# manonkok/Rao-Blackwellized-SLAM-smoothing

Hardware: AMD Instinct MI355X
Metric: particle-steps/s (filter) + smoother wall-clock, N=65k T=3k (higher is better)
Workload: dtype f64

## Files before the change

### rao-blackwellized-slam-smoothing_amd/csrc/rbpf_step_sym.hip

```cpp
#include <type_traits>
#include "rbpf_internal.hpp"
#include "rbpf_device.hpp"
#include "rbpf_model_dev.hpp"

#ifdef RBPF_STAMPS
#define RBPF_SYM_KSTAMP(k) if (blockIdx.x == 4000 && threadIdx.x == 0 && a.stamps) a.stamps[k] = __builtin_amdgcn_s_memrealtime()
#else
#define RBPF_SYM_KSTAMP(k)
#endif
#ifndef RBPF_SYM_LIGHT_WGS
#define RBPF_SYM_LIGHT_WGS 2
#endif

namespace rbpf {

typedef double dbl2s __attribute__((ext_vector_type(2)));
typedef float flt2s __attribute__((ext_vector_type(2)));
typedef float flt4s __attribute__((ext_vector_type(4)));
template <typename TS> struct SymTile { static constexpr int cg = 2; };
template <> struct SymTile<float> { static constexpr int cg = 4; };

template <typename TS> __device__ __forceinline__ dbl2s ld_tile(const TS* p);
template <> __device__ __forceinline__ dbl2s ld_tile<double>(const double* p) { return *reinterpret_cast<const dbl2s*>(p); }
template <> __device__ __forceinline__ dbl2s ld_tile<float>(const float* p) {
// ... 214 lines not shown
  constexpr int UP = UP0 * NPH > kSymStage / 2 ? kSymStage / 2 / NPH : UP0;
  constexpr int PB = (WR || UP < 4) ? 2 : 4;
  constexpr bool kCol = !(DIAG && NACT == 1);
  constexpr bool kF4 = std::is_same<TS, float>::value;
  static_assert(!kF4 || (NPH == 1 && UP % 2 == 0 && PB == 2), "fp32 tiles: whole column quads per round");
  for (int p0 = pbeg + cp; p0 < pbeg + kSymStage / 2; p0 += UP * NPH) {
    dbl2s v[UP][NACT];
    if constexpr (kF4) {
      flt4s raw[UP / 2][NACT];
#pragma unroll
      for (int j = 0; j < UP / 2; ++j)
#pragma unroll
        for (int q = 0; q < NACT; ++q) raw[j][q] = *reinterpret_cast<const flt4s*>(src[Q0 + q] + (size_t)((p0 >> 1) + j) * (4 * kSymChunk));
#pragma unroll
      for (int j = 0; j < UP / 2; ++j)
#pragma unroll
        for (int q = 0; q < NACT; ++q) {
          v[2 * j][q].x = (double)raw[j][q].x; v[2 * j][q].y = (double)raw[j][q].y;
          v[2 * j + 1][q].x = (double)raw[j][q].z; v[2 * j + 1][q].y = (double)raw[j][q].w;
        }
    } else {
#pragma unroll
    for (int u = 0; u < UP; ++u)
#pragma unroll
      for (int q = 0; q < NACT; ++q) v[u][q] = ld_tile<TS>(src[Q0 + q] + (size_t)(p0 + u * NPH) * (2 * kSymChunk));
    }
#pragma unroll
    for (int hh = 0; hh < UP / PB; ++hh) {
      double pc[PB][2][DE];
      dbl2s outv[kF4 && WR ? PB : 1][NACT];
#pragma unroll
      for (int uu = 0; uu < PB; ++uu) {
        const int u = hh * PB + uu, p = p0 + u * NPH;
        double h0[DE], h1[DE];
        {
          double hb[2 * DE + 2];
#pragma unroll
          for (int k2 = 0; k2 < (2 * DE + 1) / 2; ++k2) {
            const dbl2s t = *reinterpret_cast<const dbl2s*>(Hc + (size_t)p * 2 * DE + 2 * k2);
            hb[2 * k2] = t.x; hb[2 * k2 + 1] = t.y;
          }
#pragma unroll
          for (int k = 0; k < DE; ++k) { h0[k] = hb[k]; h1[k] = hb[DE + k]; }
        }
#pragma unroll
        for (int e = 0; e < 2; ++e)
#pragma unroll
          for (int k = 0; k < DE; ++k) pc[uu][e][k] = 0.0;
        constexpr int kChunk = 4 * D, NCH = (ND + kChunk - 1) / kChunk;
        double kc0[kChunk], kc1[kChunk];
        double pq0[NACT], pq1[NACT];
#pragma unroll
        for (int q = 0; q < NACT; ++q) { pq0[q] = v[u][q].x; pq1[q] = v[u][q].y; }
        if (WR && NCH == 1 && ND > 0) {
          double ca[D], cb[D], na[D], nb_[D];
#pragma unroll
          for (int k = 0; k < D; ++k) {
            const dbl2s t = *reinterpret_cast<const dbl2s*>(kst + ((size_t)(p % (kSymStage / 2)) * ND + k) * 2);
            ca[k] = t.x; cb[k] = t.y;
          }
#pragma unroll
          for (int s = 0; s < NS; ++s) {
            if (s + 1 < NS) {
#pragma unroll
              for (int k = 0; k < D; ++k) {
                const dbl2s t = *reinterpret_cast<const dbl2s*>(kst + ((size_t)(p % (kSymStage / 2)) * ND + (s + 1) * D + k) * 2);
                na[k] = t.x; nb_[k] = t.y;
              }
            }
#pragma unroll
            for (int q = 0; q < NACT; ++q)
#pragma unroll
              for (int k = 0; k < D; ++k) {
                pq0[q] = fma(-ks[KR == 1 ? 0 : Q0 + q][s * D + k], ca[k], pq0[q]);
                pq1[q] = fma(-ks[KR == 1 ? 0 : Q0 + q][s * D + k], cb[k], pq1[q]);
              }
            if (s + 1 < NS) {
              __builtin_amdgcn_sched_barrier(0);
#pragma unroll
              for (int k = 0; k < D; ++k) { ca[k] = na[k]; cb[k] = nb_[k]; }
            }
          }
        }
#pragma unroll
        for (int q = 0; q < NACT; ++q) {
          double p0v = pq0[q], p1v = pq1[q];
          if (WR) {
            if (NCH == 1) {
            } else {
#pragma unroll
              for (int ch = 0; ch < NCH; ++ch) {
#pragma unroll
                for (int k = 0; k < kChunk; ++k) {
                  if (ch * kChunk + k < ND) {
                    const dbl2s t = *reinterpret_cast<const dbl2s*>(kst + ((size_t)(p % (kSymStage / 2)) * ND + ch * kChunk + k) * 2);
                    kc0[k] = t.x; kc1[k] = t.y;
                  }
                }
#pragma unroll
                for (int k = 0; k < kChunk; ++k)
                  if (ch * kChunk + k < ND) {
                    p0v = fma(-ks[KR == 1 ? 0 : Q0 + q][ch * kChunk + k], kc0[k], p0v); p1v = fma(-ks[KR == 1 ? 0 : Q0 + q][ch * kChunk + k], kc1[k], p1v);
                  }
                if (ch + 1 < NCH) __builtin_amdgcn_sched_barrier(0);
              }
            }
            dbl2s o; o.x = p0v; o.y = p1v;
            if constexpr (kF4) outv[uu][q] = o;
            else st_tile<TS>(dst[Q0 + q] + (size_t)p * (2 * kSymChunk), o);
          }
#pragma unroll
          for (int k = 0; k < DE; ++k) accr[Q0 + q][k] = fma(p1v, h1[k], fma(p0v, h0[k], accr[Q0 + q][k]));
          if (!(DIAG && q == 0)) {
#pragma unroll
            for (int k = 0; k < DE; ++k) { pc[uu][0][k] = fma(p0v, hown[Q0 + q][k], pc[uu][0][k]); pc[uu][1][k] = fma(p1v, hown[Q0 + q][k], pc[uu][1][k]); }
          }
        }
      }
      if constexpr (kF4 && WR) {
#pragma unroll
        for (int q = 0; q < NACT; ++q) {
          flt4s o4; o4.x = (float)outv[0][q].x; o4.y = (float)outv[0][q].y; o4.z = (float)outv[1][q].x; o4.w = (float)outv[1][q].y;
          __builtin_nontemporal_store(o4, reinterpret_cast<flt4s*>(dst[Q0 + q] + (size_t)((p0 + hh * PB) >> 1) * (4 * kSymChunk)));
        }
      }
      if (kCol) {
        const int rho = lane >> 4;
#pragma unroll
        for (int g = 0; g < PB / 2; ++g)
#pragma unroll
          for (int k = 0; k < DE; ++k) {
            const double r = wave_sum4(pc[2 * g][0][k], pc[2 * g][1][k], pc[2 * g + 1][0][k], pc[2 * g + 1][1][k]);
            if ((lane & 15) == 0) {
              double* cq = &colp[(size_t)k * ldc + 2 * (p0 + (hh * PB + 2 * g + (rho & 1)) * NPH) + (rho >> 1)];
              *cq = ADD ? *cq + r : r;
            }
          }
      }
    }
  }
}

#ifndef RBPF_SYM_QUAD
#define RBPF_SYM_QUAD 1
#endif
#ifndef RBPF_SYM_QUAD_EMAX
#define RBPF_SYM_QUAD_EMAX 1
#endif
#ifndef RBPF_SYM_QUAD_LOADS
#define RBPF_SYM_QUAD_LOADS 16
#endif
#ifndef RBPF_SYM_BUTTERFLY
#define RBPF_SYM_BUTTERFLY 1
#endif
template <typename TS, int D, int DE, int NACT, bool DIAG, int Q0, int QL = RBPF_SYM_QUAD_LOADS>
__device__ __forceinline__ void sym_block_quad(const TS* const (&src)[kSymRows], const double* __restrict__ Hc,
                                               const double (&hown)[kSymRows][4][DE], double (&accr)[kSymRows][4][DE],
                                               double* __restrict__ colp, int ldc, int lane) {
  const int r16 = lane & 15, g = lane >> 4;
  constexpr bool kCol = !(DIAG && NACT == 1);
  constexpr int TQ = ((DE > 3 ? 8 : QL) / 4) / NACT;
  auto quad = [&](const dbl2s (&vq)[NACT][4], const int t) {
      double h0[DE], h1[DE];
      {
        double hb[2 * DE + 2];
#pragma unroll
        for (int k2 = 0; k2 < (2 * DE + 1) / 2; ++k2) {
          const dbl2s tt = *reinterpret_cast<const dbl2s*>(Hc + (size_t)(4 * t + g) * 2 * DE + 2 * k2);
          hb[2 * k2] = tt.x; hb[2 * k2 + 1] = tt.y;
        }
#pragma unroll
        for (int k = 0; k < DE; ++k) { h0[k] = hb[k]; h1[k] = hb[DE + k]; }
      }
      double pc[2][DE];
#pragma unroll
      for (int e = 0; e < 2; ++e)
#pragma unroll
        for (int k = 0; k < DE; ++k) pc[e][k] = 0.0;
#pragma unroll
      for (int q = 0; q < NACT; ++q)
#pragma unroll
        for (int rq = 0; rq < 4; ++rq) {
          const double p0v = vq[q][rq].x, p1v = vq[q][rq].y;
#pragma unroll
          for (int k = 0; k < DE; ++k) accr[Q0 + q][rq][k] = fma(p1v, h1[k], fma(p0v, h0[k], accr[Q0 + q][rq][k]));
          if (!(DIAG && q == 0)) {
#pragma unroll
            for (int k = 0; k < DE; ++k) { pc[0][k] = fma(p0v, hown[Q0 + q][rq][k], pc[0][k]); pc[1][k] = fma(p1v, hown[Q0 + q][rq][k], pc[1][k]); }
          }
        }
      if (kCol) {
        if constexpr (DE == 3 && RBPF_SYM_BUTTERFLY) {
          __builtin_amdgcn_sched_barrier(0);
          const unsigned b0 = 0u - (unsigned)(lane & 1), b1 = 0u - (unsigned)((lane >> 1) & 1);
          const double r0 = bfly_pair<0x121>(pc[0][0], pc[0][1], b0), r1 = bfly_pair<0x121>(pc[0][2], pc[1][0], b0);
          double w = bfly_pair<0x121>(pc[1][1], pc[1][2], b0);
          double q = bfly_pair<0x122>(r0, r1, b1);
          w += dpp_mov<0x122>(w);
          q += dpp_mov<0x124>(q); w += dpp_mov<0x124>(w);
          q += dpp_mov<0x128>(q); w += dpp_mov<0x128>(w);
          const int col = 2 * (4 * t + g);
          if (r16 < 4) colp[(size_t)(r16 == 3 ? 0 : r16) * ldc + col + (r16 == 3 ? 1 : 0)] = q;
          if (r16 < 2) colp[(size_t)(1 + r16) * ldc + col + 1] = w;
          __builtin_amdgcn_sched_barrier(0);
        } else {
#pragma unroll
          for (int e = 0; e < 2; ++e)
#pragma unroll
            for (int k = 0; k < DE; ++k) {
              const double r = row16_sum(pc[e][k]);
              if (r16 == 0) colp[(size_t)k * ldc + 2 * (4 * t + g) + e] = r;
            }
        }
      }
  };
#pragma unroll 1
  for (int t0 = 0; t0 < kSymChunk / 8; t0 += TQ) {
    dbl2s v[TQ][NACT][4];
#pragma unroll
    for (int u = 0; u < TQ; ++u)
#pragma unroll
      for (int q = 0; q < NACT; ++q)
#pragma unroll
        for (int rq = 0; rq < 4; ++rq)
          v[u][q][rq] = ld_tile<TS>(src[Q0 + q] + (size_t)(t0 + u) * (8 * kSymChunk) + rq * 32);
#pragma unroll
    for (int u = 0; u < TQ; ++u) quad(v[u], t0 + u);
  }
}

template <int D, int DE, int NACT, bool DIAG, int Q0>
__device__ __forceinline__ void sym_block_quad_f4(const float* const (&src)[kSymRows], const double* __restrict__ Hc,
                                                  const double (&hown)[kSymRows][4][DE], double (&accr)[kSymRows][4][DE],
                                                  double* __restrict__ colp, int ldc, int lane) {
  static_assert(DE == 3 && RBPF_SYM_BUTTERFLY, "fp32 tiles: the filter");
  const int r16 = lane & 15, g = lane >> 4;
  constexpr bool kCol = !(DIAG && NACT == 1);
#ifndef RBPF_SYM_QUAD_LOADS_F4
#define RBPF_SYM_QUAD_LOADS_F4 8
#endif
  constexpr int TQ = (RBPF_SYM_QUAD_LOADS_F4 / 4) / NACT;
#pragma unroll 1
  for (int t0 = 0; t0 < kSymChunk / 16; t0 += TQ) {
    flt4s v[TQ][NACT][4];
#pragma unroll
    for (int u = 0; u < TQ; ++u)
#pragma unroll
      for (int q = 0; q < NACT; ++q)
#pragma unroll
        for (int rq = 0; rq < 4; ++rq)
          v[u][q][rq] = *reinterpret_cast<const flt4s*>(src[Q0 + q] + (size_t)(t0 + u) * (16 * kSymChunk) + rq * 64);
#pragma unroll
    for (int u = 0; u < TQ; ++u)
#pragma unroll
      for (int h = 0; h < 2; ++h) {
        const int pi = 2 * (4 * (t0 + u) + g) + h;
        __builtin_amdgcn_sched_barrier(0);
        double h0[DE], h1[DE];
        {
          double hb[2 * DE + 2];
#pragma unroll
          for (int k2 = 0; k2 < (2 * DE + 1) / 2; ++k2) {
            const dbl2s tt = *reinterpret_cast<const dbl2s*>(Hc + (size_t)pi * 2 * DE + 2 * k2);
            hb[2 * k2] = tt.x; hb[2 * k2 + 1] = tt.y;
          }
#pragma unroll
          for (int k = 0; k < DE; ++k) { h0[k] = hb[k]; h1[k] = hb[DE + k]; }
        }
        double pc[2][DE];
#pragma unroll
        for (int e = 0; e < 2; ++e)
#pragma unroll
          for (int k = 0; k < DE; ++k) pc[e][k] = 0.0;
#pragma unroll
        for (int q = 0; q < NACT; ++q)
#pragma unroll
          for (int rq = 0; rq < 4; ++rq) {
            const double p0v = (double)(h ? v[u][q][rq].z : v[u][q][rq].x), p1v = (double)(h ? v[u][q][rq].w : v[u][q][rq].y);
#pragma unroll
            for (int k = 0; k < DE; ++k) accr[Q0 + q][rq][k] = fma(p1v, h1[k], fma(p0v, h0[k], accr[Q0 + q][rq][k]));
            if (!(DIAG && q == 0)) {
#pragma unroll
              for (int k = 0; k < DE; ++k) { pc[0][k] = fma(p0v, hown[Q0 + q][rq][k], pc[0][k]); pc[1][k] = fma(p1v, hown[Q0 + q][rq][k], pc[1][k]); }
            }
          }
        if (kCol) {
          __builtin_amdgcn_sched_barrier(0);
          const unsigned b0 = 0u - (unsigned)(lane & 1), b1 = 0u - (unsigned)((lane >> 1) & 1);
          const double r0 = bfly_pair<0x121>(pc[0][0], pc[0][1], b0), r1 = bfly_pair<0x121>(pc[0][2], pc[1][0], b0);
          double w = bfly_pair<0x121>(pc[1][1], pc[1][2], b0);
          double q = bfly_pair<0x122>(r0, r1, b1);
          w += dpp_mov<0x122>(w);
          q += dpp_mov<0x124>(q); w += dpp_mov<0x124>(w);
          q += dpp_mov<0x128>(q); w += dpp_mov<0x128>(w);
          const int col = 2 * pi;
          if (r16 < 4) colp[(size_t)(r16 == 3 ? 0 : r16) * ldc + col + (r16 == 3 ? 1 : 0)] = q;
          if (r16 < 2) colp[(size_t)(1 + r16) * ldc + col + 1] = w;
          __builtin_amdgcn_sched_barrier(0);
        }
      }
  }
}

template <typename TS, int D, int NS, bool WR, int E, int CH>
__device__ __forceinline__ void step_sym_body(const StepArgs& a) {
#include "rbpf_step_sym_body.inc"
// ... 156 lines not shown
```

### rao-blackwellized-slam-smoothing_amd/csrc/rbpf_step_sym_body.inc

```
  const int chv = CH ? CH : a.lay.CH64;
  const int NW = sym_waves(chv), NT = 64 * NW;
  constexpr int NPH = sym_phases(CH);
  constexpr bool kGStrip = (CH == 16 || CH == 0);
  extern __shared__ double smem[];
  constexpr int DE = D + E, ND = NS * D, NDA = ND > 0 ? ND : 1, NSA = NS > 0 ? NS : 1;
  constexpr bool kSplit = WR && NS > 4;
  const ModelDev& M = a.mdl;
  const Layout& Ly = a.lay;
  const int n = Ly.n, nb = Ly.nb, mc = Ly.mc, ldx = Ly.ldx, ldb = Ly.ldb;
  const int pos = xcd_position((int)blockIdx.x, (int)gridDim.x);
  const int* pre_i = a.pre_i + (size_t)pos * kPreInts;
  if (a.phase >= 0 && pre_i[5] != a.phase) return;
  const int i = pre_i[0];
  const int dslot = WR ? pre_i[4] : i;
  const int tid = threadIdx.x, lane = tid & 63, wave = tid >> 6;
  const SymPlan lp = sym_plan(n, DE, ldx, M.ktot, WR ? ND : 0, chv, ((RBPF_SYM_LIGHT_WGS > 2 && !WR && E == 0) || kGStrip) ? 0 : 1);
  double* Hs = smem + lp.off_H + ((nb * DE) & 1);
  double* xls = smem + lp.off_xl;
  double* PHt = smem + lp.off_PHt;
  double* tabS = smem + lp.off_tab;
  double* tabC = tabS + (M.ktot > 0 ? M.ktot : 1);
  double* misc = smem + lp.off_misc;
  double* red = smem + lp.off_red;
#ifdef RBPF_SYM_DIAG_SAMEBASE
  const int ancb = pre_i[2], baseb = pre_i[3] & 63;
#else
  const int ancb = pre_i[2], baseb = pre_i[3];
#endif
  const bool remote = a.rec != nullptr && ancb >= a.n_bank_local;
  const double* recp = remote ? a.rec + (size_t)(ancb - a.n_bank_local) * a.rec_stride : nullptr;
  const bool remoteP = a.rec != nullptr && baseb >= a.n_bank_local;
  const double* recP = remoteP ? a.rec + (size_t)(baseb - a.n_bank_local) * a.rec_stride : nullptr;
  const TS* srcT = remoteP ? reinterpret_cast<const TS*>(recP) : reinterpret_cast<const TS*>(a.Pt_old) + (size_t)baseb * a.Pt_old_stride;
  const TS* srcB = remoteP ? reinterpret_cast<const TS*>(recP + a.rec_off_B) : reinterpret_cast<const TS*>(a.Pb_old) + (size_t)baseb * a.Pb_old_stride;
  const double* srcX = remote ? recp + a.rec_off_X : a.xl_old + (size_t)ancb * a.xl_old_stride;
  const double* Fs[NSA];
#pragma unroll
  for (int s = 0; s < NSA; ++s) Fs[s] = nullptr;
#pragma unroll
  for (int s = 0; s < NS; ++s) {
    if (a.fset[s]) Fs[s] = a.fset[s] + (size_t)pre_i[kPreSet0 + s] * 2 * D * ldx;
    else Fs[s] = remote ? recp + a.rec_off_F : a.F_old + (size_t)ancb * 2 * D * ldx;
  }

  RBPF_SYM_KSTAMP(0);
  const double* pre_d = a.pre_d + (size_t)pos * kPreDoubles;
  const double px0 = pre_d[0], px1 = pre_d[1], px2 = pre_d[2];
  constexpr int kNNPre = 2;
  const int crot = (M.kind == 1) ? 3 : 0;
  auto jcol = [&](int ci) { const int c = ci + crot; return c >= n ? c - n : c; };
  int nnp[kNNPre][3] = {};
  if (a.H_ext == nullptr) {
#pragma unroll
    for (int it = 0; it < kNNPre; ++it)
      if (tid + it * NT < n) H_column_indices(M, jcol(tid + it * NT), nnp[it]);
  }
  constexpr bool kCorr = !WR && NS > 0;
  constexpr int kFPre = NS > 6 ? 2 : 3, kSPre = kFPre;
  double kvp[kCorr ? kFPre : 1][NDA], ksp[kCorr ? kSPre : 1][NDA];
  if constexpr (kCorr) {
#pragma unroll
    for (int it = 0; it < kFPre; ++it)
      if (tid + it * NT < n) {
#pragma unroll
        for (int s = 0; s < NS; ++s)
#pragma unroll
          for (int k = 0; k < D; ++k) kvp[it][s * D + k] = Fs[s][(size_t)(D + k) * ldx + tid + it * NT];
      }
  }
  if (tid < kPreDoubles) misc[tid] = pre_d[tid];
  constexpr bool kXlLds = !(RBPF_SYM_LIGHT_WGS > 2 && !WR && E == 0) && !kGStrip;
  if (kXlLds) for (int c = tid; c < n; c += NT) xls[c] = srcX[c];
  double Riy[D];
  if (E > 0) {
    const double* iv = remote ? recp + a.rec_off_I : a.ivec_old + (size_t)ancb * a.ivec_old_stride;
    for (int c = tid; c < n; c += NT) Hs[c * DE + D] = iv[c];
#pragma unroll
    for (int aa = 0; aa < D; ++aa) {
      double sacc = 0.0;
#pragma unroll
      for (int bb = 0; bb < D; ++bb) sacc = fma(M.Rinv[aa + D * bb], a.y[bb], sacc);
      Riy[aa] = sacc;
    }
  }
  RBPF_SYM_KSTAMP(1);
  for (int q = tid; q < M.ktot; q += NT) basis_table_entry(M, q, px0, px1, px2, tabS, tabC);
  __syncthreads();
  RBPF_SYM_KSTAMP(2);
  {
    auto column = [&](int c, const int* nn) {
      double h[D];
      if (a.H_ext != nullptr) {
#pragma unroll
        for (int k = 0; k < D; ++k) h[k] = a.H_ext[((size_t)i * D + k) * ldx + c];
      } else {
        H_column<D>(M, c, nn, tabS, tabC, &misc[8], h);
      }
#pragma unroll
      for (int k = 0; k < D; ++k) Hs[c * DE + k] = h[k];
      if (E > 0) {
        double sp = Hs[c * DE + D];
#pragma unroll
        for (int k = 0; k < D; ++k) sp = fma(h[k], Riy[k], sp);
#pragma unroll
        for (int k = 0; k < D; ++k) a.Hb_new[((size_t)i * D + k) * ldx + c] = h[k];
        a.ivec_new[(size_t)i * ldx + c] = sp;
      }
    };
#pragma unroll
    for (int it = 0; it < kNNPre; ++it)
      if (tid + it * NT < n) column(jcol(tid + it * NT), nnp[it]);
    for (int ci = tid + kNNPre * NT; ci < n; ci += NT) {
      int nn[3] = {0, 0, 0};
      if (a.H_ext == nullptr) H_column_indices(M, jcol(ci), nn);
      column(jcol(ci), nn);
    }
  }
  __syncthreads();
  if constexpr (kCorr) {
    constexpr int NG = NS * D * DE;
    double g[NG];
#pragma unroll
    for (int q = 0; q < NG; ++q) g[q] = 0.0;
    auto gcol = [&](int c, const double* kv) {
      double h[DE];
#pragma unroll
      for (int k = 0; k < DE; ++k) h[k] = Hs[c * DE + k];
#pragma unroll
      for (int s = 0; s < NS; ++s)
#pragma unroll
        for (int k = 0; k < D; ++k)
#pragma unroll
          for (int j = 0; j < DE; ++j) g[(s * D + k) * DE + j] = fma(kv[s * D + k], h[j], g[(s * D + k) * DE + j]);
    };
#pragma unroll
    for (int it = 0; it < kFPre; ++it)
      if (tid + it * NT < n) gcol(tid + it * NT, kvp[it]);
    for (int c = tid + kFPre * NT; c < n; c += NT) {
      double kv[NDA];
#pragma unroll
      for (int s = 0; s < NS; ++s)
#pragma unroll
        for (int k = 0; k < D; ++k) kv[s * D + k] = Fs[s][(size_t)(D + k) * ldx + c];
      gcol(c, kv);
    }
    wave_sums_packed<NG>(g, lane, [&](int q, double s) { red[wave * kSymRed + q] = s; });
  }

  RBPF_SYM_KSTAMP(3);
  {
  const int rp = (NPH == 1) ? wave : (wave % (chv / 2)), cp = (NPH == 1) ? 0 : (wave / (chv / 2));
  const int rows[kSymRows] = {rp, chv - 1 - rp};
  constexpr bool kQuad = RBPF_SYM_QUAD && !WR && NPH == 1 && E <= RBPF_SYM_QUAD_EMAX;
  constexpr int kQL = CH == 0 ? 8 : RBPF_SYM_QUAD_LOADS;
  double accr[kSymRows][DE], hown[kSymRows][DE], ks[kSplit ? 1 : kSymRows][NDA];
  double accq[kQuad ? kSymRows : 1][4][DE], hq[kQuad ? kSymRows : 1][4][DE];
  if constexpr (kQuad) {
#pragma unroll
    for (int q = 0; q < kSymRows; ++q)
#pragma unroll
      for (int rq = 0; rq < 4; ++rq)
#pragma unroll
        for (int k = 0; k < DE; ++k) { accq[q][rq][k] = 0.0; hq[q][rq][k] = Hs[(nb + rows[q] * kSymChunk + 16 * rq + (lane & 15)) * DE + k]; }
  }
#pragma unroll
  for (int q = 0; q < kSymRows; ++q) {
    const int r = nb + rows[q] * kSymChunk + lane;
#pragma unroll
    for (int k = 0; k < DE; ++k) { accr[q][k] = 0.0; hown[q][k] = Hs[r * DE + k]; }
#pragma unroll
    for (int s = 0; s < NS; ++s)
#pragma unroll
      for (int k = 0; k < D; ++k) ks[kSplit ? 0 : q][s * D + k] = (WR && !kSplit) ? Fs[s][(size_t)k * ldx + r] : 0.0;
    for (int b = 0; b < nb && cp == 0 && !kQuad; ++b) {
      double pv = (double)srcB[(size_t)b * ldb + r];
      if (WR) {
#pragma unroll
        for (int sset = 0; sset < NS; ++sset)
#pragma unroll
          for (int k = 0; k < D; ++k) pv = fma(-Fs[sset][(size_t)k * ldx + b], Fs[sset][(size_t)(D + k) * ldx + r], pv);
      }
#pragma unroll
      for (int k = 0; k < DE; ++k) accr[q][k] = fma(pv, Hs[b * DE + k], accr[q][k]);
    }
  }
  if (WR) __syncthreads();
  {
    TS* dT = reinterpret_cast<TS*>(a.Pt_new) + (size_t)dslot * Ly.szT;
    double* kst = smem + lp.off_kst + (size_t)wave * kSymStage * ND;
    double* colw = (rp == 0) ? PHt + nb : (kGStrip ? smem + lp.off_col1 + (size_t)wave * DE * kSymChunk : smem + sym_off_col(lp.off_col1, DE, chv, rp));
    const int ldc = (rp == 0) ? ldx : (kGStrip ? kSymChunk : sym_ld_col(chv, rp));
    double* gstrip = kGStrip ? a.strip_ws + (size_t)blockIdx.x * a.strip_ws_stride + sym_off_col(0, DE, chv, rp) : nullptr;
    const double* Hcore = Hs + (size_t)nb * DE;
    double kpre[NDA];
    auto fetch = [&](int col0) {
#pragma unroll
      for (int s = 0; s < NS; ++s)
#pragma unroll
        for (int k = 0; k < D; ++k) kpre[s * D + k] = Fs[s][(size_t)(D + k) * ldx + col0 + (lane & (kSymStage - 1))];
    };
    auto park = [&]() {
      asm volatile("" ::: "memory");
      if (lane < kSymStage) {
#pragma unroll
        for (int k = 0; k < ND; ++k) kst[((size_t)(lane >> 1) * ND + k) * 2 + (lane & 1)] = kpre[k];
      }
      asm volatile("" ::: "memory");
    };
    const int last = rows[kSymRows - 1];
    for (int J = 0; J <= last; ++J) {
      const TS* src[kSymRows]; TS* dst[kSymRows];
#pragma unroll
      for (int q = 0; q < kSymRows; ++q) {
        const size_t off = ((size_t)rows[q] * (rows[q] + 1) / 2 + J) * kSymTile + SymTile<TS>::cg * lane;
        src[q] = srcT + off; dst[q] = dT + off;
      }
      const double* Hc = Hcore + (size_t)J * kSymChunk * DE;
      double* colp = (kGStrip && rp > 0) ? colw : colw + (size_t)J * kSymChunk;
      if constexpr (kQuad) {
        const TS* srq[kSymRows];
#pragma unroll
        for (int q = 0; q < kSymRows; ++q)
          srq[q] = srcT + ((size_t)rows[q] * (rows[q] + 1) / 2 + J) * kSymTile + SymTile<TS>::cg * (kSymChunk * (lane >> 4) + (lane & 15));
        if constexpr (std::is_same<TS, float>::value) {
          if (J < rows[0]) sym_block_quad_f4<D, DE, 2, false, 0>(srq, Hc, hq, accq, colp, ldc, lane);
          else if (J == rows[0]) sym_block_quad_f4<D, DE, 2, true, 0>(srq, Hc, hq, accq, colp, ldc, lane);
          else if (J < last) sym_block_quad_f4<D, DE, 1, false, 1>(srq, Hc, hq, accq, colp, ldc, lane);
          else sym_block_quad_f4<D, DE, 1, true, 1>(srq, Hc, hq, accq, colp, ldc, lane);
        } else {
        if (J < rows[0]) sym_block_quad<TS, D, DE, 2, false, 0, kQL>(srq, Hc, hq, accq, colp, ldc, lane);
        else if (J == rows[0]) sym_block_quad<TS, D, DE, 2, true, 0, kQL>(srq, Hc, hq, accq, colp, ldc, lane);
        else if (J < last) sym_block_quad<TS, D, DE, 1, false, 1, kQL>(srq, Hc, hq, accq, colp, ldc, lane);
        else sym_block_quad<TS, D, DE, 1, true, 1, kQL>(srq, Hc, hq, accq, colp, ldc, lane);
        }
      } else if constexpr (!kSplit) {
        for (int pbeg = 0; pbeg < kSymChunk / 2; pbeg += kSymStage / 2) {
          if (WR && ND > 0) { fetch(nb + J * kSymChunk + 2 * pbeg); park(); }
          if (J < rows[0]) sym_block<TS, D, DE, NS, WR, 2, false, 0, false, kSymRows, NPH>(src, dst, Hc, kst, pbeg, cp, ks, hown, accr, colp, ldc, lane);
          else if (J == rows[0]) sym_block<TS, D, DE, NS, WR, 2, true, 0, false, kSymRows, NPH>(src, dst, Hc, kst, pbeg, cp, ks, hown, accr, colp, ldc, lane);
          else if (J < last) sym_block<TS, D, DE, NS, WR, 1, false, 1, false, kSymRows, NPH>(src, dst, Hc, kst, pbeg, cp, ks, hown, accr, colp, ldc, lane);
          else sym_block<TS, D, DE, NS, WR, 1, true, 1, false, kSymRows, NPH>(src, dst, Hc, kst, pbeg, cp, ks, hown, accr, colp, ldc, lane);
        }
      } else {
#pragma unroll
        for (int s = 0; s < NS; ++s)
#pragma unroll
          for (int k = 0; k < D; ++k) ks[0][s * D + k] = Fs[s][(size_t)k * ldx + nb + rows[1] * kSymChunk + lane];
        for (int pbeg = 0; pbeg < kSymChunk / 2; pbeg += kSymStage / 2) {
          fetch(nb + J * kSymChunk + 2 * pbeg); park();
          if (J < last) sym_block<TS, D, DE, NS, WR, 1, false, 1, false, 1, NPH>(src, dst, Hc, kst, pbeg, cp, ks, hown, accr, colp, ldc, lane);
          else sym_block<TS, D, DE, NS, WR, 1, true, 1, false, 1, NPH>(src, dst, Hc, kst, pbeg, cp, ks, hown, accr, colp, ldc, lane);
        }
        if (J <= rows[0]) {
#pragma unroll
          for (int s = 0; s < NS; ++s)
#pragma unroll
            for (int k = 0; k < D; ++k) ks[0][s * D + k] = Fs[s][(size_t)k * ldx + nb + rows[0] * kSymChunk + lane];
          for (int pbeg = 0; pbeg < kSymChunk / 2; pbeg += kSymStage / 2) {
            fetch(nb + J * kSymChunk + 2 * pbeg); park();
            if (J < rows[0]) sym_block<TS, D, DE, NS, WR, 1, false, 0, true, 1, NPH>(src, dst, Hc, kst, pbeg, cp, ks, hown, accr, colp, ldc, lane);
            else sym_block<TS, D, DE, NS, WR, 1, true, 0, true, 1, NPH>(src, dst, Hc, kst, pbeg, cp, ks, hown, accr, colp, ldc, lane);
          }
        }
      }
      if (kGStrip && rp > 0 && J < last) {
#pragma unroll
        for (int k = 0; k < DE; ++k) gstrip[(size_t)k * sym_ld_col(chv, rp) + J * kSymChunk + lane] = colw[k * kSymChunk + lane];
      }
    }
  }
  if constexpr (kCorr) {
    int tq = tid;
    asm volatile("" : "+v"(tq));
#pragma unroll
    for (int it = 0; it < kSPre; ++it)
      if (tq + it * NT < n) {
#pragma unroll
        for (int s = 0; s < NS; ++s)
#pragma unroll
          for (int k = 0; k < D; ++k) ksp[it][s * D + k] = Fs[s][(size_t)k * ldx + tq + it * NT];
      }
  }
  constexpr int kBPre = 4;
  double pvp[kQuad ? kSymRows : 1][kBPre];
  if constexpr (kQuad) {
#pragma unroll
    for (int q = 0; q < kSymRows; ++q)
#pragma unroll
      for (int b = 0; b < kBPre; ++b)
        if (b < nb) pvp[q][b] = (double)srcB[(size_t)b * ldb + nb + sym_quad_row(rows[q], lane)];
  }
  RBPF_SYM_KSTAMP(7);
  for (int b = wave; b < nb; b += NW) {
    const TS* src = srcB + (size_t)b * ldb;
    TS* dstb = reinterpret_cast<TS*>(a.Pb_new) + (size_t)dslot * Ly.szB + (size_t)b * ldb;
    double ksb[NDA];
#pragma unroll
    for (int s = 0; s < NS; ++s)
#pragma unroll
      for (int k = 0; k < D; ++k) ksb[s * D + k] = WR ? Fs[s][(size_t)k * ldx + b] : 0.0;
    double accb[DE];
#pragma unroll
    for (int k = 0; k < DE; ++k) accb[k] = 0.0;
    for (int c = 2 * lane; c < ldb; c += 128) {
      const dbl2s vv = ld_tile<TS>(src + c);
      double p[2] = {vv.x, vv.y};
#pragma unroll
      for (int e = 0; e < 2; ++e) {
        const int cc = c + e;
        if (cc < n) {
          if (WR) {
#pragma unroll
            for (int s = 0; s < NS; ++s)
#pragma unroll
              for (int k = 0; k < D; ++k) p[e] = fma(-ksb[s * D + k], Fs[s][(size_t)(D + k) * ldx + cc], p[e]);
          }
#pragma unroll
          for (int k = 0; k < DE; ++k) accb[k] = fma(p[e], Hs[cc * DE + k], accb[k]);
        }
      }
      if (WR) { dbl2s o; o.x = p[0]; o.y = p[1]; st_tile<TS>(dstb + c, o); }
    }
    if constexpr (D > 1) {
      wave_sums_packed<DE>(accb, lane, [&](int k, double s) { PHt[(size_t)k * ldx + b] = s; });
    } else {
#pragma unroll
      for (int k = 0; k < DE; ++k) {
        const double s = wave_sum(accb[k]);
        if (lane == 0) PHt[(size_t)k * ldx + b] = s;
      }
    }
  }
  if (NPH > 1 && cp > 0) {
    double* rowp = smem + lp.off_row + (size_t)(cp - 1) * DE * chv * kSymChunk;
#pragma unroll
    for (int q = 0; q < kSymRows; ++q)
#pragma unroll
      for (int k = 0; k < DE; ++k) rowp[(size_t)k * (chv * kSymChunk) + rows[q] * kSymChunk + lane] = accr[q][k];
  }
  __syncthreads();
  if (cp == 0) {
#pragma unroll
    for (int q = 0; q < kSymRows; ++q) {
      const int rc = kQuad ? sym_quad_row(rows[q], lane) : rows[q] * kSymChunk + lane;
      double s[DE];
#pragma unroll
      for (int k = 0; k < DE; ++k) s[k] = accr[q][k];
      if constexpr (kQuad) {
#pragma unroll
        for (int k = 0; k < DE; ++k) s[k] = 0.0;
#pragma unroll
        for (int b = 0; b < kBPre; ++b)
          if (b < nb) {
#pragma unroll
            for (int k = 0; k < DE; ++k) s[k] = fma(pvp[q][b], Hs[b * DE + k], s[k]);
          }
        for (int b = kBPre; b < nb; ++b) {
          const double pv = (double)srcB[(size_t)b * ldb + nb + rc];
#pragma unroll
          for (int k = 0; k < DE; ++k) s[k] = fma(pv, Hs[b * DE + k], s[k]);
        }
#pragma unroll
        for (int k = 0; k < DE; ++k)
          s[k] = fold16(fold32(accq[q][0][k], accq[q][1][k]), fold32(accq[q][2][k], accq[q][3][k])) + s[k];
      }
      if (NPH > 1) {
#pragma unroll
        for (int ph = 1; ph < NPH; ++ph) {
          const double* rowp = smem + lp.off_row + (size_t)(ph - 1) * DE * chv * kSymChunk;
#pragma unroll
          for (int k = 0; k < DE; ++k) s[k] += rowp[(size_t)k * (chv * kSymChunk) + rc];
        }
      }
#pragma unroll
      for (int w = 0; w < chv / 2; ++w) {
        if (rows[q] < chv - 1 - w) {
          const double* cw = (w == 0) ? PHt + nb : (kGStrip ? a.strip_ws + (size_t)blockIdx.x * a.strip_ws_stride + sym_off_col(0, DE, chv, w)
                                                            : smem + sym_off_col(lp.off_col1, DE, chv, w));
          const int ldw = (w == 0) ? ldx : sym_ld_col(chv, w);
#pragma unroll
          for (int k = 0; k < DE; ++k) s[k] += cw[(size_t)k * ldw + rc];
        }
      }
#pragma unroll
      for (int k = 0; k < DE; ++k) PHt[(size_t)k * ldx + nb + rc] = s[k];
    }
  }
  __syncthreads();
  }
  if (!WR && NS > 0) {
    constexpr int NG = NS * D * DE > 0 ? NS * D * DE : 1;
    double g[NG];
#pragma unroll
    for (int q = 0; q < NG; ++q) {
      double s = red[q];
      for (int w = 1; w < NW; ++w) s += red[w * kSymRed + q];
      g[q] = s;
    }
    auto corr = [&](int r, const double* ksr) {
      double ph[DE];
#pragma unroll
      for (int j = 0; j < DE; ++j) ph[j] = PHt[(size_t)j * ldx + r];
#pragma unroll
      for (int s = 0; s < NS; ++s)
#pragma unroll
        for (int k = 0; k < D; ++k)
#pragma unroll
          for (int j = 0; j < DE; ++j) ph[j] = fma(-ksr[s * D + k], g[(s * D + k) * DE + j], ph[j]);
#pragma unroll
      for (int j = 0; j < DE; ++j) PHt[(size_t)j * ldx + r] = ph[j];
    };
#pragma unroll
    for (int it = 0; it < kSPre; ++it)
      if (tid + it * NT < n) corr(tid + it * NT, ksp[kCorr ? it : 0]);
    int tq = tid;
    asm volatile("" : "+v"(tq));
    for (int r = tq + kSPre * NT; r < n; r += NT) {
      double ksr[NDA];
#pragma unroll
      for (int s = 0; s < NS; ++s)
#pragma unroll
        for (int k = 0; k < D; ++k) ksr[s * D + k] = Fs[s][(size_t)k * ldx + r];
      corr(r, ksr);
    }
    __syncthreads();
  }

  RBPF_SYM_KSTAMP(4);
  constexpr int NRED = D * D + D + 2 * E;
  {
    double part[NRED];
#pragma unroll
    for (int q = 0; q < NRED; ++q) part[q] = 0.0;
    for (int r = tid; r < n; r += NT) {
      double h[D], ph[D];
#pragma unroll
      for (int k = 0; k < D; ++k) { h[k] = Hs[r * DE + k]; ph[k] = PHt[(size_t)k * ldx + r]; }
      const double x = kXlLds ? xls[r] : srcX[r];
#pragma unroll
      for (int bb = 0; bb < D; ++bb)
#pragma unroll
        for (int aa = 0; aa < D; ++aa) part[aa + D * bb] = fma(h[aa], ph[bb], part[aa + D * bb]);
#pragma unroll
      for (int aa = 0; aa < D; ++aa) part[D * D + aa] = fma(h[aa], x, part[D * D + aa]);
      if (E > 0) {
        const double iv = Hs[r * DE + D], piv = PHt[(size_t)D * ldx + r];
        double ivp = iv, pivp = piv;
#pragma unroll
        for (int k = 0; k < D; ++k) { ivp = fma(h[k], Riy[k], ivp); pivp = fma(ph[k], Riy[k], pivp); }
        part[D * D + D] = fma(iv, piv, part[D * D + D]);
        part[D * D + D + 1] = fma(ivp, pivp, part[D * D + D + 1]);
      }
    }
    wave_sums_packed<NRED>(part, lane, [&](int q, double s) { red[wave * kSymRed + q] = s; });
  }
  __syncthreads();
  if (wave == 0) {
    double sq = 0.0;
    if (lane < NRED) {
      sq = red[lane];
      for (int w = 1; w < NW; ++w) sq += red[w * kSymRed + lane];
    }
    double SS[D * D], e[D], cS[D * D] = {}, v[D];
#pragma unroll
    for (int q = 0; q < D * D; ++q) SS[q] = sym_lane_read(sq, q) + M.R[q];
#pragma unroll
    for (int q = 0; q < D; ++q) e[q] = a.y[q] - sym_lane_read(sq, D * D + q);
    bool ok = chol_lower_small<D>(SS, cS);
    if (!ok) {
      double SJ[D * D];
      for (int q = 0; q < D * D; ++q) SJ[q] = SS[q];
      for (int q = 0; q < D; ++q) SJ[q + D * q] += M.jitter;
      ok = chol_lower_small<D>(SJ, cS);
    }
    double dg = cS[0];
#pragma unroll
    for (int q = 1; q < D; ++q) dg = (lane == q) ? cS[q + D * q] : dg;
    const double lg = log(dg);
    double lgq[D];
#pragma unroll
    for (int q = 0; q < D; ++q) lgq[q] = sym_lane_read(lg, q);
    double lw = 0.0, sl = 0.0;
    if (ok) {
      fwd_subst<D>(cS, e, v);
      double vv = 0.0;
      for (int q = 0; q < D; ++q) { sl += lgq[q]; vv += v[q] * v[q]; }
      lw = -sl - 0.5 * vv + M.logconst;
    } else {
      lw = nan("");
      for (int q = 0; q < D * D; ++q) cS[q] = 0.0;
      for (int q = 0; q < D; ++q) cS[q + D * q] = 1.0;
    }
    if (lane == 0) {
      if (!ok) atomicOr(a.status, 1);
      if (E == 0) a.logw[i] = lw;
      for (int q = 0; q < D * D; ++q) { misc[20 + q] = cS[q]; misc[30 + q] = SS[q]; }
      for (int q = 0; q < D; ++q) misc[40 + q] = e[q];
    }
    if (E > 0) {
      const double qa = sym_lane_read(sq, D * D + D), qb = sym_lane_read(sq, D * D + D + 1);
      if (lane == 0) { misc[44] = qa; misc[45] = qb; misc[46] = ok ? sl : nan(""); }
    }
  }
  __syncthreads();

  RBPF_SYM_KSTAMP(5);
  {
    double cS[D * D], SS[D * D], e[D];
#pragma unroll
    for (int q = 0; q < D * D; ++q) { cS[q] = misc[20 + q]; SS[q] = misc[30 + q]; }
#pragma unroll
    for (int q = 0; q < D; ++q) e[q] = misc[40 + q];
    double* KSn = a.F_new + ((size_t)i * 2 + 0) * D * ldx;
    double* Kn = a.F_new + ((size_t)i * 2 + 1) * D * ldx;
    if (tid == 0) {
      if (a.base_new) a.base_new[i] = WR ? dslot : (a.share_flush ? pre_i[4] : baseb);
      if (!WR) {
#pragma unroll
        for (int s = 0; s < NS; ++s)
          if (a.fset_idx_new[s]) a.fset_idx_new[s][i] = pre_i[kPreSet0 + s];
      }
      if (a.fself_idx_new) a.fself_idx_new[i] = i;
    }
    double* xln = a.xl_new + (size_t)i * ldx;
    double uK[D];
#pragma unroll
    for (int k = 0; k < D; ++k) uK[k] = 0.0;
    for (int r = tid; r < n; r += NT) {
      double ph[D], u[D], kk[D];
#pragma unroll
      for (int k = 0; k < D; ++k) ph[k] = PHt[(size_t)k * ldx + r];
      fwd_subst<D>(cS, ph, u);
      bwd_subst_T<D>(cS, u, kk);
      double xn_ = kXlLds ? xls[r] : srcX[r];
#pragma unroll
      for (int k = 0; k < D; ++k) xn_ = fma(kk[k], e[k], xn_);
      xln[r] = xn_;
#pragma unroll
      for (int j = 0; j < D; ++j) {
        double s = 0.0;
#pragma unroll
        for (int k = 0; k < D; ++k) s = fma(kk[k], SS[k + D * j], s);
        KSn[(size_t)j * ldx + r] = s;
// ... 40 lines not shown
```

Before: 6.187 million.

## Move border-row PHt reduction to the front and fuse correction into finalize

Border-row products (P_b·H) are now computed before the symmetric main pass, with the first tiles of the border rows prefetched into registers at kernel entry so their latency overlaps the setup work. For small NS with D>1, the rank correction of PHt is fused into the per-row finalize step using register-held F rows. This removes a separate pass with an extra barrier and a second read and write of PHt. The cost is higher register pressure from the brp/ksc/ksbr arrays, which could reduce occupancy.

```diff
diff --git a/rao-blackwellized-slam-smoothing_amd/csrc/rbpf_step_sym.hip b/rao-blackwellized-slam-smoothing_amd/csrc/rbpf_step_sym.hip
--- a/rao-blackwellized-slam-smoothing_amd/csrc/rbpf_step_sym.hip
+++ b/rao-blackwellized-slam-smoothing_amd/csrc/rbpf_step_sym.hip
@@ -390,6 +390,12 @@
 #endif
 #ifndef RBPF_SYM_BUTTERFLY
 #define RBPF_SYM_BUTTERFLY 1
+#endif
+#ifndef RBPF_SYM_BORDER_FRONT
+#define RBPF_SYM_BORDER_FRONT 1
+#endif
+#ifndef RBPF_SYM_FUSE_CORR
+#define RBPF_SYM_FUSE_CORR 4
 #endif
 template <typename TS, int D, int DE, int NACT, bool DIAG, int Q0, int QL = RBPF_SYM_QUAD_LOADS>
 __device__ __forceinline__ void sym_block_quad(const TS* const (&src)[kSymRows], const double* __restrict__ Hc,
diff --git a/rao-blackwellized-slam-smoothing_amd/csrc/rbpf_step_sym_body.inc b/rao-blackwellized-slam-smoothing_amd/csrc/rbpf_step_sym_body.inc
--- a/rao-blackwellized-slam-smoothing_amd/csrc/rbpf_step_sym_body.inc
+++ b/rao-blackwellized-slam-smoothing_amd/csrc/rbpf_step_sym_body.inc
@@ -57,7 +57,18 @@
   }
   constexpr bool kCorr = !WR && NS > 0;
   constexpr int kFPre = NS > 6 ? 2 : 3, kSPre = kFPre;
-  double kvp[kCorr ? kFPre : 1][NDA], ksp[kCorr ? kSPre : 1][NDA];
+  constexpr bool kBFront = RBPF_SYM_BORDER_FRONT && !WR && D > 1;
+  constexpr bool kFuse = kCorr && D > 1 && NS <= RBPF_SYM_FUSE_CORR;
+  double kvp[kCorr ? kFPre : 1][NDA], ksp[(kCorr && !kFuse) ? kSPre : 1][NDA];
+  constexpr int kBRPre = 5;
+  dbl2s brp[kBFront ? kBRPre : 1];
+  if constexpr (kBFront) {
+    if (wave < nb) {
+#pragma unroll
+      for (int it = 0; it < kBRPre; ++it)
+        if (2 * lane + 128 * it < ldb) brp[it] = ld_tile<TS>(srcB + (size_t)wave * ldb + 2 * lane + 128 * it);
+    }
+  }
   if constexpr (kCorr) {
 #pragma unroll
     for (int it = 0; it < kFPre; ++it)
@@ -145,6 +156,40 @@
       gcol(c, kv);
     }
     wave_sums_packed<NG>(g, lane, [&](int q, double s) { red[wave * kSymRed + q] = s; });
+  }
+  if constexpr (kBFront) {
+    for (int b = wave; b < nb; b += NW) {
+      const TS* src = srcB + (size_t)b * ldb;
+      double accb[DE];
+#pragma unroll
+      for (int k = 0; k < DE; ++k) accb[k] = 0.0;
+      auto bround = [&](int c, const dbl2s vv) {
+        const double p[2] = {vv.x, vv.y};
+#pragma unroll
+        for (int e = 0; e < 2; ++e) {
+          const int cc = c + e;
+          if (cc < n) {
+#pragma unroll
+            for (int k = 0; k < DE; ++k) accb[k] = fma(p[e], Hs[cc * DE + k], accb[k]);
+          }
+        }
+      };
+      if (b == wave) {
+#pragma unroll
+        for (int it = 0; it < kBRPre; ++it)
+          if (2 * lane + 128 * it < ldb) bround(2 * lane + 128 * it, brp[it]);
+      }
+      for (int c = 2 * lane + (b == wave ? 128 * kBRPre : 0); c < ldb; c += 128) bround(c, ld_tile<TS>(src + c));
+      if constexpr (D > 1) {
+        wave_sums_packed<DE>(accb, lane, [&](int k, double s) { PHt[(size_t)k * ldx + b] = s; });
+      } else {
+#pragma unroll
+        for (int k = 0; k < DE; ++k) {
+          const double s = wave_sum(accb[k]);
+          if (lane == 0) PHt[(size_t)k * ldx + b] = s;
+        }
+      }
+    }
   }
 
   RBPF_SYM_KSTAMP(3);
@@ -269,7 +314,28 @@
       }
     }
   }
-  if constexpr (kCorr) {
+  double ksc[kFuse ? kSymRows : 1][NDA], ksbr[NDA];
+  if constexpr (kFuse) {
+    int lq = lane;
+    asm volatile("" : "+v"(lq));
+    if (cp == 0) {
+#pragma unroll
+      for (int q = 0; q < kSymRows; ++q) {
+        const int r = nb + (kQuad ? sym_quad_row(rows[q], lq) : rows[q] * kSymChunk + lq);
+#pragma unroll
+        for (int s = 0; s < NS; ++s)
+#pragma unroll
+          for (int k = 0; k < D; ++k) ksc[q][s * D + k] = Fs[s][(size_t)k * ldx + r];
+      }
+    }
+    if (wave * 64 + lq < nb) {
+#pragma unroll
+      for (int s = 0; s < NS; ++s)
+#pragma unroll
+        for (int k = 0; k < D; ++k) ksbr[s * D + k] = Fs[s][(size_t)k * ldx + wave * 64 + lq];
+    }
+  }
+  if constexpr (kCorr && !kFuse) {
     int tq = tid;
     asm volatile("" : "+v"(tq));
 #pragma unroll
@@ -291,7 +357,7 @@
         if (b < nb) pvp[q][b] = (double)srcB[(size_t)b * ldb + nb + sym_quad_row(rows[q], lane)];
   }
   RBPF_SYM_KSTAMP(7);
-  for (int b = wave; b < nb; b += NW) {
+  for (int b = kBFront ? nb : wave; b < nb; b += NW) {
     const TS* src = srcB + (size_t)b * ldb;
     TS* dstb = reinterpret_cast<TS*>(a.Pb_new) + (size_t)dslot * Ly.szB + (size_t)b * ldb;
     double ksb[NDA];
@@ -339,11 +405,12 @@
       for (int k = 0; k < DE; ++k) rowp[(size_t)k * (chv * kSymChunk) + rows[q] * kSymChunk + lane] = accr[q][k];
   }
   __syncthreads();
+  double sfin[kFuse ? kSymRows : 1][DE];
   if (cp == 0) {
 #pragma unroll
     for (int q = 0; q < kSymRows; ++q) {
       const int rc = kQuad ? sym_quad_row(rows[q], lane) : rows[q] * kSymChunk + lane;
-      double s[DE];
+      double (&s)[DE] = sfin[kFuse ? q : 0];
 #pragma unroll
       for (int k = 0; k < DE; ++k) s[k] = accr[q][k];
       if constexpr (kQuad) {
@@ -382,13 +449,54 @@
           for (int k = 0; k < DE; ++k) s[k] += cw[(size_t)k * ldw + rc];
         }
       }
-#pragma unroll
-      for (int k = 0; k < DE; ++k) PHt[(size_t)k * ldx + nb + rc] = s[k];
+      if constexpr (!kFuse) {
+#pragma unroll
+        for (int k = 0; k < DE; ++k) PHt[(size_t)k * ldx + nb + rc] = s[k];
+      }
+    }
+  }
+  constexpr int NGC = kFuse ? NS * D * DE : 1;
+  double gc[NGC];
+  if constexpr (kFuse) {
+    __builtin_amdgcn_sched_barrier(0);
+#pragma unroll
+    for (int q = 0; q < NGC; ++q) {
+      double s = red[q];
+      for (int w = 1; w < NW; ++w) s += red[w * kSymRed + q];
+      gc[q] = s;
+    }
+    __builtin_amdgcn_sched_barrier(0);
+  }
+  auto corr_reg = [&](double (&ph)[DE], const double (&ksr)[NDA]) {
+#pragma unroll
+    for (int s = 0; s < NS; ++s)
+#pragma unroll
+      for (int k = 0; k < D; ++k)
+#pragma unroll
+        for (int j = 0; j < DE; ++j) ph[j] = fma(-ksr[s * D + k], gc[kFuse ? (s * D + k) * DE + j : 0], ph[j]);
+  };
+  if constexpr (kFuse) {
+    if (cp == 0) {
+#pragma unroll
+      for (int q = 0; q < kSymRows; ++q) {
+        const int rc = kQuad ? sym_quad_row(rows[q], lane) : rows[q] * kSymChunk + lane;
+        corr_reg(sfin[q], ksc[q]);
+#pragma unroll
+        for (int k = 0; k < DE; ++k) PHt[(size_t)k * ldx + nb + rc] = sfin[q][k];
+      }
+    }
+    if (tid < nb) {
+      double ph[DE];
+#pragma unroll
+      for (int j = 0; j < DE; ++j) ph[j] = PHt[(size_t)j * ldx + tid];
+      corr_reg(ph, ksbr);
+#pragma unroll
+      for (int j = 0; j < DE; ++j) PHt[(size_t)j * ldx + tid] = ph[j];
     }
   }
   __syncthreads();
   }
-  if (!WR && NS > 0) {
+  if constexpr (kCorr && !kFuse) {
     constexpr int NG = NS * D * DE > 0 ? NS * D * DE : 1;
     double g[NG];
 #pragma unroll
```

After: 6.146 million. Within noise of the previous version (-0.7%).
